# moyun/deneva

Measured on AMD Instinct MI355X. Metric: OCC-validated txns/sec, YCSB theta=0.9, higher is better.
Workload: dtype u64; 1 GPU; YCSB OCC epoch validation, 1048576 txns x 16 keys, zipf theta=0.9, 16,777,216-key table, 50% RO txns, 50% WR tuples; global_batch=1048576, keys_per_txn=16, parallelism=single GPU

## Files before the change

### deneva_amd/csrc/occ_sweep.hip

```cpp
#include <hip/hip_runtime.h>

#include <algorithm>

#include "dcc_device.h"
#include "occ_kernels.h"
#include "prep_body.h"

namespace dcc {

constexpr uint32_t LB_ACC_BITS = 34;

__device__ inline uint32_t sw_hash(uint64_t key, uint32_t log2s) {
  const uint32_t h = (uint32_t)key * 0x9E3779B1u ^ (uint32_t)(key >> 32) * 0x85EBCA77u;
  return h >> (32 - log2s);
}

__device__ inline uint32_t gtab_step(uint64_t key, uint32_t gbits, uint32_t step) {
  const uint32_t h = sw_hash(key, gbits);
  const uint32_t nbm = (1u << (gbits - 2)) - 1u;
  const uint32_t b = ((h >> 2) + (step >> 2)) & nbm;
  return 4 * b + (((h & 3u) + step) & 3u);
}
__device__ inline unsigned long long gtab_cas(uint64_t* gt, uint32_t slot, uint64_t key) {
  return atomicCAS((unsigned long long*)(gt + slot), (unsigned long long)KEY_EMPTY,
// ... 599 lines not shown
      while (true) {
        if (lds_ld(&s_stop)) {
          stopped = true;
          break;
        }
        if (lds_ld(&s_done) + SEQ_RING > k) break;
        pw++;
        __builtin_amdgcn_s_sleep(8);
      }
      if (stopped) break;
      const uint4* src = (const uint4*)(a.rec + k);
      uint4* dst = (uint4*)&ring[slot];
      uint4 v[SEQ_V4 / 64];
#pragma unroll
      for (uint32_t q = 0; q < SEQ_V4 / 64; q++) v[q] = src[q * 64 + lane];
#pragma unroll
      for (uint32_t q = 0; q < SEQ_V4 / 64; q++) dst[q * 64 + lane] = v[q];
      if (lane == 0) lds_st(&s_ready[slot], k + 1);
    }
    if (dbg && lane == 0 && pw) atomicAdd((unsigned long long*)&dbg[7], (unsigned long long)pw);
  } else if (ntiles) {
    uint32_t k = 0, cw = 0, st_it = 0;
    uint64_t st_u = 0;
    __builtin_amdgcn_s_setprio(3);
    const uint64_t cyc0 = __builtin_amdgcn_s_memtime();
    while (lds_ld(&s_ready[0]) != 1u) {
      cw++;
      __builtin_amdgcn_s_sleep(1);
    }
    uint64_t cdep, cseg[SW_RC];
    uint32_t cmeta, chdr, cpe[SW_RC], cie[SW_RC_I];
    auto read_rec = [&](const SwRec& T) {
      cdep = T.dep[lane];
      cmeta = T.meta[lane];
      chdr = T.hdr;
#pragma unroll
      for (uint32_t c = 0; c < SW_RC; c++) {
        cpe[c] = T.probe[c * 64 + lane];
        cseg[c] = T.seg[c][lane];
      }
#pragma unroll
      for (uint32_t c = 0; c < SW_RC_I; c++) cie[c] = T.ins[c * 64 + lane];
    };
    read_rec(ring[0]);
    if (ntiles > 1)
      while (lds_ld(&s_ready[1 % SEQ_RING]) != 2u) {
        cw++;
        __builtin_amdgcn_s_sleep(1);
      }
    uint32_t fl = 0, slot = 0;
    for (; k < ntiles; k++) {
      const uint32_t hdr = __builtin_amdgcn_readfirstlane(chdr);
      if (hdr & SWH_STOP) break;
      const uint64_t dep = cdep;
      const uint32_t meta = cmeta;
      uint64_t seg[SW_RC];
      uint32_t pe[SW_RC], ie[SW_RC_I];
#pragma unroll
      for (uint32_t c = 0; c < SW_RC; c++) {
        seg[c] = cseg[c];
        pe[c] = cpe[c];
      }
#pragma unroll
      for (uint32_t c = 0; c < SW_RC_I; c++) ie[c] = cie[c];
      const uint32_t kn = k + 1, sn = slot + 1 == SEQ_RING ? 0u : slot + 1;
      uint32_t h[SW_RC];
#pragma unroll
      for (uint32_t c = 0; c < SW_RC; c++) h[c] = cb_probe(cbits, pe[c]);
      read_rec(ring[sn]);
      fl = lds_ld_rlx(&s_ready[sn + 1 == SEQ_RING ? 0u : sn + 1]);
      uint64_t kv = 0;
#pragma unroll
      for (uint32_t c = 0; c < SW_RC; c++) kv |= ballot64(h[c] != 0) & seg[c];
      uint64_t K = ballot64(kv != 0);
      if (hdr & SWH_PLONG) {
        const uint32_t np = __builtin_amdgcn_readfirstlane(ring[slot].np);
        const uint32_t sp = ring[slot].pspan[lane];
        const uint32_t ps = sp & 0xFFFFu, pe2 = sp >> 16;
        const uint32_t* ovf = a.lst_ovf + (uint64_t)k * SW_OVF;
        bool kill = false;
        for (uint32_t q0 = SW_RC * 64; q0 < np; q0 += 64) {
          const uint32_t q = q0 + lane;
          uint32_t e = SW_P_NONE;
          if (q < np) e = q < SW_PL ? ring[slot].probe[q] : ld_sync(ovf + (q - SW_PL));
          kill |= seg_any(ballot64(cb_probe(cbits, e) != 0), ps, pe2, q0);
        }
        K |= ballot64(kill);
      }
      uint64_t U = ballot64((meta & (SWM_VALID | SWM_PRE)) == SWM_VALID) & ~K, M = 0;
      st_u += __builtin_popcountll(U);
      if (U) {
        const uint64_t d = ballot64((dep & U) == 0);
        M = U & d;
        U &= ~d;
        while (U) {
          const uint64_t cm = U & ballot64((dep & (M | U)) == 0);
          const uint64_t am = U & ballot64((dep & M) != 0);
          M |= cm;
          U &= ~(cm | am);
          st_it++;
        }
      }
      if (kn + 1 < ntiles)
        while (fl != kn + 2) {
          cw++;
          __builtin_amdgcn_s_sleep(1);
          fl = lds_ld_rlx(&s_ready[sn + 1 == SEQ_RING ? 0u : sn + 1]);
        }
      __atomic_signal_fence(__ATOMIC_SEQ_CST);
#pragma unroll
      for (uint32_t c = 0; c < SW_RC_I; c++) cb_insert_m(cbits, ie[c], M);
      if (hdr & SWH_ILONG) {
        const uint32_t ni = __builtin_amdgcn_readfirstlane(ring[slot].ni);
        const uint32_t* ovf = a.lst_ovf + (uint64_t)k * SW_OVF;
        for (uint32_t q0 = SW_RC_I * 64; q0 < ni; q0 += 64) {
          const uint32_t q = q0 + lane;
          uint32_t e = sw_idummy(lane);
          if (q < ni) e = q < SW_IL ? ring[slot].ins[q] : ld_sync(ovf + SW_TA + (q - SW_IL));
          cb_insert_m(cbits, e, M);
        }
      }
      s_M[k] = M;
      __hip_atomic_store(&s_done, kn, __ATOMIC_RELAXED, __HIP_MEMORY_SCOPE_WORKGROUP);
      slot = sn;
    }
    if (lane == 0) {
      s_k = k;
      lds_st(&s_stop, 1u);
      if (dbg) {
        dbg[2] = __builtin_amdgcn_s_memrealtime();
        dbg[5] = cw;
        dbg[6] = k;
        dbg[8] = __builtin_amdgcn_s_memtime() - cyc0;
        dbg[9] = st_u;
        dbg[10] = st_it;
      }
    }
  }
  __syncthreads();
  const uint32_t k = s_k;
  constexpr uint32_t WO_U = 8;
  for (uint32_t q0 = 0; q0 < k * SW_T; q0 += SEQ_B * WO_U) {
    uint32_t mt[WO_U], tid[WO_U];
#pragma unroll
    for (uint32_t u = 0; u < WO_U; u++) {
      const uint32_t q = q0 + u * SEQ_B + j;
      mt[u] = 0;
      tid[u] = 0;
      if (q < k * SW_T) {
        mt[u] = a.rec[q / SW_T].meta[q % SW_T];
        tid[u] = a.rec[q / SW_T].rtid[q % SW_T];
      }
    }
    bool cw[WO_U];
#pragma unroll
    for (uint32_t u = 0; u < WO_U; u++) {
      const uint32_t q = q0 + u * SEQ_B + j;
      cw[u] = false;
      if (mt[u] & SWM_VALID) {
        const bool com = (s_M[q / SW_T] >> (q % SW_T)) & 1ull;
        if (!(mt[u] & SWM_PRE)) a.state[tid[u]] = com ? ST_COMMIT : ST_ABORT;
        if (a.write_hasw) a.hasw[tid[u]] = (mt[u] & SWM_HASW) ? 1 : 0;
        cw[u] = com && !(mt[u] & SWM_PRE) && (mt[u] & SWM_HASW);
      }
    }
    if (a.cw_list) {
      uint64_t bm[WO_U];
      uint32_t tot = 0;
#pragma unroll
      for (uint32_t u = 0; u < WO_U; u++) {
        bm[u] = ballot64(cw[u]);
        tot += (uint32_t)__popcll(bm[u]);
      }
      uint32_t base = 0;
      if (lane == 0 && tot) base = atomicAdd(a.cw_count, tot);
      base = __shfl(base, 0);
#pragma unroll
      for (uint32_t u = 0; u < WO_U; u++) {
        if (cw[u]) a.cw_list[base + (uint32_t)__popcll(bm[u] & lanemask_lt())] = tid[u];
        base += (uint32_t)__popcll(bm[u]);
      }
    }
  }
  if (dbg) {
    __syncthreads();
    if (j == 0) dbg[3] = __builtin_amdgcn_s_memrealtime();
  }
  for (uint32_t q = j; q < k; q += SEQ_B) a.mg[q] = s_M[q];
  for (uint32_t q = j; q < nwords; q += SEQ_B) a.cbits_out[q] = 0;
  for (uint32_t q = j; q < (1u << SW_BLOOM_LOG) / 32; q += SEQ_B) a.bloom_out[q] = 0;
  if (j == 0) {
    a.lv->pos = min(k * SW_T, lim);
    a.lv->ccount = 0;
    if (dbg) dbg[4] = __builtin_amdgcn_s_memrealtime();
  }
}

__global__ __launch_bounds__(256) void k_sw_cout(SwCoutArgs a) {
  __shared__ uint32_t s_cnt[4];
  __shared__ uint32_t s_base;
  if (blockIdx.x >= a.cout_grid) {
    const uint32_t b = blockIdx.x - a.cout_grid, nb = gridDim.x - a.cout_grid;
    prep_body_hasw(a.prep_off, a.prep_n, a.prep_at, a.prep_nnz, a.hasw, a.prep_part, b, nb, a.prep_err);
    const uint4 e = make_uint4(~0u, ~0u, ~0u, ~0u);
    for (uint64_t q = (uint64_t)b * 256 + threadIdx.x; q < a.wclear_n16; q += (uint64_t)nb * 256)
      a.wclear[q] = e;
    return;
  }
  const uint32_t ab = *a.abandon;
  const uint32_t pos = a.lv->pos;
  const uint32_t m = list_len(a.m_dev, a.m_host);
  const uint32_t o0_raw = a.in.off[0];
  if (ab) return;
  if (a.skip_done && pos >= m) return;
  const uint32_t lane = lane_id(), wv = threadIdx.x >> 6;
  const uint64_t nnz = a.in.nnz;
  const uint32_t off0 = (uint32_t)min((uint64_t)o0_raw, nnz);
  const uint32_t range = (uint32_t)min((uint64_t)a.in.off[pos], nnz) - off0;
  for (uint32_t x0 = blockIdx.x * 1024; x0 < range; x0 += gridDim.x * 1024) {
    uint32_t ent[4], ap[4];
    uint64_t kx[4];
    bool c[4];
#pragma unroll
    for (uint32_t u = 0; u < 4; u++) {
      const uint32_t x = x0 + wv * 256 + u * 64 + lane;
      const bool in = x < range;
      ent[u] = in ? a.aent[x] : 0u;
      ap[u] = in ? a.apos[x] : 0u;
      kx[u] = in ? a.in.keys[off0 + x] : 0ull;
    }
    uint64_t mw[4];
#pragma unroll
    for (uint32_t u = 0; u < 4; u++) mw[u] = (ent[u] & 32u) ? a.mg[ap[u] >> 6] : 0ull;
#pragma unroll
    for (uint32_t u = 0; u < 4; u++) c[u] = (ent[u] & 32u) && ((mw[u] >> (ap[u] & 63u)) & 1ull);
    uint64_t cm[4];
    uint32_t wc = 0;
#pragma unroll
    for (uint32_t u = 0; u < 4; u++) {
      cm[u] = ballot64(c[u]);
      wc += (uint32_t)__popcll(cm[u]);
    }
    if (lane == 0) s_cnt[wv] = wc;
    __syncthreads();
    if (threadIdx.x == 0) {
      const uint32_t tot = s_cnt[0] + s_cnt[1] + s_cnt[2] + s_cnt[3];
      s_base = tot ? atomicAdd(&a.lv->ccount, tot) : 0u;
    }
    __syncthreads();
    uint32_t base = s_base;
    for (uint32_t w = 0; w < wv; w++) base += s_cnt[w];
#pragma unroll
    for (uint32_t u = 0; u < 4; u++) {
      if (c[u]) {
        const uint64_t key = kx[u];
        a.ckeys_out[base + (uint32_t)__popcll(cm[u] & lanemask_lt())] = key;
        const uint32_t id = sw_aid(ent[u]);
        if (id < SW_ID_NONE) atomicOr(&a.cbits_out[id >> 5], 1u << (id & 31u));
        uint32_t b1, b2;
        bloom_bits(key, b1, b2);
        atomicOr(&a.bloom_out[b1 >> 5], 1u << (b1 & 31));
        atomicOr(&a.bloom_out[b2 >> 5], 1u << (b2 & 31));
      }
      base += (uint32_t)__popcll(cm[u]);
    }
    __syncthreads();
  }
}


constexpr uint32_t FW = SW_CHUNK / 64;
constexpr uint32_t FK = 16;
constexpr uint32_t SW_CMP_MAXR = 4096;

__device__ inline bool c_exact(const SwFilterArgs& a, uint64_t key) {
  const uint32_t nbm = (1u << (a.gbits - 2)) - 1u;
  uint32_t b = sw_hash(key, a.gbits - 2);
  for (uint32_t q = 0; q <= nbm; q++) {
    const uint4* p = (const uint4*)(a.gtab + 4 * (uint64_t)b);
    const uint4 x = p[0], y = p[1];
    const uint32_t nib = (a.cbits[b >> 3] >> ((b & 7u) * 4u)) & 15u;
    const uint64_t v0 = ((uint64_t)x.y << 32) | x.x, v1 = ((uint64_t)x.w << 32) | x.z;
    const uint64_t v2 = ((uint64_t)y.y << 32) | y.x, v3 = ((uint64_t)y.w << 32) | y.z;
    if (v0 == key) return nib & 1u;
    if (v1 == key) return (nib >> 1) & 1u;
    if (v2 == key) return (nib >> 2) & 1u;
    if (v3 == key) return (nib >> 3) & 1u;
    if (v0 == KEY_EMPTY || v1 == KEY_EMPTY || v2 == KEY_EMPTY || v3 == KEY_EMPTY) return false;
    b = (b + 1) & nbm;
  }
  return false;
}
constexpr uint32_t F_STASH = 256;
#ifndef DCC_F_XS
#define DCC_F_XS 2048
#endif
#ifndef DCC_F_WPE
#define DCC_F_WPE 1
#endif
constexpr uint32_t F_XS = DCC_F_XS;
constexpr uint32_t F_XCAP = F_XS / 2;
constexpr uint32_t F_XBITS_LOG = 16;

__global__ __launch_bounds__(SW_CHUNK, DCC_F_WPE) void k_sw_filter(SwFilterArgs a) {
  constexpr uint32_t B = SW_CHUNK, FW = B / 64;
  constexpr uint32_t CS = F_XS;
  struct XSet {
    uint32_t bl[(1u << F_XBITS_LOG) / 32];
    uint64_t cex[F_XS];
  };
  union FSet {
    XSet x;
    uint32_t bl[(1u << SW_BLOOM_LOG) / 32];
  };
  __shared__ __attribute__((aligned(16))) FSet fs;
  uint32_t* const bl = fs.bl;
  uint64_t* const cex = fs.x.cex;
  __shared__ uint64_t s_hit[FW][SW_WA / 64];
  __shared__ uint64_t s_stash[FW][F_STASH];
  __shared__ uint32_t s_wpre[FW][SW_WA / 64];
  const uint32_t j = threadIdx.x, lane = lane_id(), wv = j >> 6;
  const uint32_t ab = *a.abandon;
  const uint32_t m = list_len(a.m_dev, a.m_host);
  const uint32_t pos = a.lv->pos;
  const uint32_t ccount = a.lv->ccount;
  if (ab) return;
  const bool X = ccount <= F_XCAP;
  uint64_t* dbg = (a.dbg && blockIdx.x < 256 && j == 0) ? a.dbg + 8 * blockIdx.x : nullptr;
  if (dbg) dbg[0] = __builtin_amdgcn_s_memrealtime();
  if (pos >= m && !a.kill_out) return;
  for (uint64_t q = (uint64_t)blockIdx.x * B + j; q < a.gclear_n;
       q += (uint64_t)gridDim.x * B) {
    a.gclear[q] = KEY_EMPTY;
    a.fw_clear[q] = ~0u;
    a.la_clear[q] = 0u;
  }
  if (pos >= m) return;
  const uint32_t n64 = (m - pos + 63) / 64;
  const uint64_t nnz = a.in.nnz;
  const uint32_t R = sw_tiles_per_wg(n64, gridDim.x);
  const uint32_t t_lo = min(blockIdx.x * R, n64), t_hi = min(t_lo + R, n64);
  if (t_lo >= t_hi) {
    if (!a.kill_out && j == 0) {
      a.bsum[blockIdx.x] = 0;
      if (a.ro_split) a.rbsum[blockIdx.x] = 0;
    }
    return;
  }
  const bool small = X;
  {
    if (!X) {
      const uint4* src = (const uint4*)a.bloom;
      uint4* dst = (uint4*)bl;
      for (uint32_t q = j; q < (1u << SW_BLOOM_LOG) / 128; q += B) dst[q] = src[q];
    } else {
      for (uint32_t q = j; q < (1u << F_XBITS_LOG) / 32; q += B) bl[q] = 0;
      for (uint32_t q = j; q < CS; q += B) cex[q] = KEY_EMPTY;
    }
  }
  __syncthreads();
  if (small) {
    for (uint32_t q = j; q < ccount; q += B) {
      const uint64_t kq = a.ckeys[q];
      lset_insert<CS>(cex, kq);
      if (X) {
        uint32_t b1, b2;
        bloom_bits(kq, b1, b2);
        b1 >>= SW_BLOOM_LOG - F_XBITS_LOG;
        atomicOr(&bl[b1 >> 5], 1u << (b1 & 31u));
      }
    }
    __syncthreads();
  }
  if (dbg) dbg[1] = __builtin_amdgcn_s_memrealtime();
  uint64_t* hit = s_hit[wv];
  uint64_t* stash = s_stash[wv];
  uint64_t wsum = 0, rsum = 0;
  uint32_t ns = 0, ne = 0, ntid = 0, nst = 0, nhw = 1;
  auto prefetch = [&](uint32_t wt) {
    const uint32_t pc = min(pos + wt * 64 + lane, m - 1);
    ns = a.in.off[pc];
    ne = a.in.off[pc + 1];
    ntid = a.in.tid ? a.in.tid[pc] : pc;
    nst = a.cand_state ? a.state[pc] : 0u;
    if (a.ro_split) nhw = a.hasw[pc];
  };
  if (t_lo + wv < t_hi) prefetch(t_lo + wv);
  for (uint32_t wt = t_lo + wv; wt < t_hi; wt += FW) {
    const uint32_t p = pos + wt * 64 + lane;
    const bool valid = p < m;
    uint32_t s = 0, e = 0, tid = 0;
    bool cand = false, ro = false;
    if (valid) {
      s = (uint32_t)min((uint64_t)ns, nnz);
      e = (uint32_t)min((uint64_t)ne, nnz);
      if (e < s) e = s;
      tid = ntid;
      cand = nst == ST_UNDECIDED;
      ro = nhw == 0;
    }
    bool pref = false;
    const uint64_t vm = ballot64(valid);
    const uint32_t A0 = vm ? __shfl(s, 0) : 0u;
    const uint32_t A1 = wave_reduce<MaxOp<uint32_t>>(valid ? e : 0u);
    uint32_t span = A1 > A0 ? A1 - A0 : 0u;
    if (span > SW_WA) {
      if (lane == 0) atomicOr(a.err, ERR_TILE);
      span = 0;
    }
    const uint32_t nw = (span + 63) / 64;
    uint32_t npos = 0;
    bool bad_key = false;
    for (uint32_t b0 = 0; b0 < span; b0 += 64 * FK) {
      uint64_t key[FK];
#pragma unroll
      for (uint32_t u = 0; u < FK; u++) {
        const uint32_t xr = b0 + 64 * u + lane;
        const uint32_t x = A0 + (xr < span ? xr : 0u);
        key[u] = a.in.keys[x];
      }
      if (!pref) {
        pref = true;
        if (wt + FW < t_hi) prefetch(wt + FW);
      }
#pragma unroll
      for (uint32_t u = 0; u < FK; u++) {
        const uint32_t xr = b0 + 64 * u + lane;
        if (b0 + 64 * u >= span) continue;
        const bool in = xr < span;
        bad_key |= in && key[u] == KEY_EMPTY;
        bool h;
        uint32_t b1, b2;
        bloom_bits(key[u], b1, b2);
        if (X) {
          b1 >>= SW_BLOOM_LOG - F_XBITS_LOG;
          h = in && ((bl[b1 >> 5] >> (b1 & 31u)) & 1u) != 0;
        } else {
          const uint32_t wa = bl[b1 >> 5], wb = bl[b2 >> 5];
          h = in && (((wa >> (b1 & 31u)) & (wb >> (b2 & 31u)) & 1u) != 0);
        }
        const uint64_t hb = ballot64(h);
        if (h) {
          const uint32_t ci = npos + (uint32_t)__popcll(hb & lanemask_lt());
          if (ci < F_STASH) stash[ci] = key[u];
        }
        npos += (uint32_t)__popcll(hb);
        if (lane == 0) hit[(b0 >> 6) + u] = hb;
      }
    }
    if (!pref && wt + FW < t_hi) prefetch(wt + FW);
    if (ballot64(bad_key) && lane == 0) atomicOr(a.err, ERR_KEY);
    if (dbg && wt == t_lo) dbg[2] = __builtin_amdgcn_s_memrealtime();
    const uint32_t rlo = s - A0, rlen = e - s;
    const bool ok = valid && (rlen == 0 || (uint64_t)rlo + rlen <= span);
    bool killed = false;
    {
      {
        const uint32_t pw = lane < nw ? (uint32_t)__popcll(hit[lane]) : 0u;
        uint32_t ptot;
        const uint32_t pre = wave_excl<AddOp<uint32_t>>(pw, ptot);
        if (lane < nw) s_wpre[wv][lane] = pre;
      }
      if (cand && ok && rlen) {
        for (uint32_t x = rlo; x < rlo + rlen; x++) {
          const uint32_t nx = range_next(hit, x, rlo + rlen);
          if (nx >= rlo + rlen) break;
          const uint32_t ci = s_wpre[wv][nx >> 6] +
                              (uint32_t)__popcll(hit[nx >> 6] & ((1ull << (nx & 63)) - 1ull));
          const uint64_t kx = ci < F_STASH ? stash[ci] : a.in.keys[A0 + nx];
          if (small ? lset_find<CS>(cex, kx) : c_exact(a, kx)) {
            killed = true;
            break;
          }
          x = nx;
        }
      }
    }
    if (dbg && wt == t_lo) dbg[3] = __builtin_amdgcn_s_memrealtime();
    if (dbg) dbg[6]++;
    if (a.kill_out) {
      const uint64_t km = ballot64(valid && killed);
      if (lane == 0) a.kill_out[wt] = km;
      continue;
    }
    if (killed) a.state[tid] = ST_ABORT;
    if (cand && ok && rlen == 0) a.state[tid] = ST_COMMIT;
    const bool surv = cand && ok && rlen && !killed;
    const uint64_t sm = ballot64(surv);
    const uint64_t acc = wave_reduce<AddOp<uint64_t>>(surv ? rlen : 0u);
    const uint64_t cnt = ((uint64_t)__popcll(sm) << LB_ACC_BITS) | acc;
    wsum += cnt;
    if (lane == 0) {
      a.sflag[wt] = sm;
      a.tcount[wt] = cnt;
    }
    if (a.ro_split) {
      const uint64_t rm = ballot64(surv && ro);
      const uint64_t racc = wave_reduce<AddOp<uint64_t>>(surv && ro ? rlen : 0u);
      const uint64_t rc = ((uint64_t)__popcll(rm) << LB_ACC_BITS) | racc;
      rsum += rc;
      if (lane == 0) {
        a.rflag[wt] = rm;
        a.rtcount[wt] = rc;
      }
    }
    if (dbg && wt == t_lo) {
      __builtin_amdgcn_s_waitcnt(0);
      dbg[4] = __builtin_amdgcn_s_memrealtime();
    }
  }
  if (a.kill_out) return;
  __shared__ unsigned long long s_bs[FW][2];
  if (lane == 0) {
    s_bs[wv][0] = wsum;
    s_bs[wv][1] = rsum;
  }
  __syncthreads();
  if (j == 0) {
    uint64_t t = 0, r = 0;
    for (uint32_t w = 0; w < FW; w++) {
      t += s_bs[w][0];
      r += s_bs[w][1];
    }
    a.bsum[blockIdx.x] = t;
    if (a.ro_split) a.rbsum[blockIdx.x] = r;
  }
  if (dbg) {
    __builtin_amdgcn_s_waitcnt(0);
    dbg[5] = __builtin_amdgcn_s_memrealtime();
  }
}

__global__ __launch_bounds__(SW_CHUNK) void k_sw_apply(SwFilterArgs a) {
  const uint32_t lane = lane_id(), wv = threadIdx.x >> 6;
  if (*a.abandon) return;
  const uint32_t m = list_len(a.m_dev, a.m_host);
  const uint32_t pos = a.lv->pos;
  if (pos >= m) return;
  const uint32_t n64 = (m - pos + 63) / 64;
  const uint64_t nnz = a.in.nnz;
  const uint32_t R = sw_tiles_per_wg(n64, gridDim.x);
  const uint32_t t_lo = min(blockIdx.x * R, n64), t_hi = min(t_lo + R, n64);
  uint64_t wsum = 0, rsum = 0;
  for (uint32_t wt = t_lo + wv; wt < t_hi; wt += SW_CHUNK / 64) {
    const uint32_t p = pos + wt * 64 + lane;
    uint64_t kw = 0;
    for (uint32_t r = 0; r < a.kill_ranks; r++) kw |= a.kill_in[r * a.kill_stride + wt];
    const bool kill = (kw >> lane) & 1ull;
    bool surv = false, ro = false;
    uint32_t len = 0;
    if (p < m) {
      const uint32_t tid = a.in.tid ? a.in.tid[p] : p;
      const bool cand = a.cand_state ? a.state[p] == ST_UNDECIDED : true;
      const uint32_t s = (uint32_t)min((uint64_t)a.in.off[p], nnz);
      const uint32_t e = (uint32_t)min((uint64_t)a.in.off[p + 1], nnz);
      len = e > s ? e - s : 0u;
      if (cand && kill) a.state[tid] = ST_ABORT;
      surv = cand && !kill;
      ro = a.ro_split && a.hasw[tid] == 0;
    }
    const uint64_t sm = ballot64(surv);
    const uint64_t acc = wave_reduce<AddOp<uint64_t>>(surv ? len : 0u);
    const uint64_t cnt = ((uint64_t)__popcll(sm) << LB_ACC_BITS) | acc;
    wsum += cnt;
    if (lane == 0) {
      a.sflag[wt] = sm;
      a.tcount[wt] = cnt;
    }
    if (a.ro_split) {
      const uint64_t rm = ballot64(surv && ro);
      const uint64_t racc = wave_reduce<AddOp<uint64_t>>(surv && ro ? len : 0u);
      const uint64_t rc = ((uint64_t)__popcll(rm) << LB_ACC_BITS) | racc;
      rsum += rc;
      if (lane == 0) {
        a.rflag[wt] = rm;
        a.rtcount[wt] = rc;
      }
    }
  }
  __shared__ unsigned long long s_bs[SW_CHUNK / 64][2];
  if (lane == 0) {
    s_bs[wv][0] = wsum;
    s_bs[wv][1] = rsum;
  }
  __syncthreads();
  if (threadIdx.x == 0) {
    uint64_t t = 0, r = 0;
    for (uint32_t w = 0; w < SW_CHUNK / 64; w++) {
      t += s_bs[w][0];
      r += s_bs[w][1];
    }
    a.bsum[blockIdx.x] = t;
    if (a.ro_split) a.rbsum[blockIdx.x] = r;
  }
}

constexpr uint32_t SG_T = 1024;
__global__ __launch_bounds__(SG_T) void k_sw_sg_scan(const uint32_t* tid, const uint32_t* m_dev, uint32_t p_max,
                                                     const uint32_t* full_off, uint64_t full_nnz, uint32_t* soff,
                                                     uint32_t* err) {
  __shared__ uint32_t s_w[SG_T / 64];
  __shared__ uint32_t s_carry;
  const uint32_t P = min(p_max, *m_dev);
  if (threadIdx.x == 0) s_carry = 0;
  __syncthreads();
  for (uint32_t q0 = 0; q0 < P; q0 += SG_T) {
    const uint32_t q = q0 + threadIdx.x;
    uint32_t len = 0;
    if (q < P) {
      const uint32_t t = tid[q];
      const uint64_t s = min((uint64_t)full_off[t], full_nnz), e = min((uint64_t)full_off[t + 1], full_nnz);
      len = e > s ? (uint32_t)(e - s) : 0u;
      if (len > MAX_TXN_LEN) {
        atomicOr(err, ERR_OFFSETS);
        len = 0;
      }
    }
    uint32_t tot;
    const uint32_t ex = s_carry + block_excl<SG_T / 64, AddOp<uint32_t>>(len, s_w, tot);
    if (q < P) soff[q] = ex;
    __syncthreads();
    if (threadIdx.x == SG_T - 1) s_carry = ex + len;
    __syncthreads();
  }
  if (threadIdx.x == 0) soff[P] = s_carry;
}
__global__ __launch_bounds__(256) void k_sw_sg_copy(const uint32_t* tid, const uint32_t* m_dev, uint32_t p_max,
                                                    const uint32_t* full_off, const uint64_t* full_keys,
                                                    const uint8_t* full_at, uint64_t full_nnz, const uint32_t* soff,
                                                    uint64_t* skeys, uint8_t* sat) {
  const uint32_t P = min(p_max, *m_dev), sl = threadIdx.x & 15u;
  for (uint32_t q = (blockIdx.x * 256 + threadIdx.x) >> 4; q < P; q += gridDim.x * 16) {
    const uint32_t t = tid[q], o = soff[q], len = soff[q + 1] - o;
    const uint64_t s = min((uint64_t)full_off[t], full_nnz);
    for (uint32_t x = sl; x < len; x += 16) {
      skeys[o + x] = full_keys[s + x];
      sat[o + x] = full_at[s + x];
    }
  }
}

__global__ void k_sw_share(const uint32_t* m_dev, uint32_t m_host, const uint32_t* abandon,
                           const uint32_t* off, uint32_t p_max, uint32_t rank, uint32_t* cnt) {
  const uint32_t m = m_dev ? *m_dev : m_host;
  const uint32_t P = min(p_max, m);
  cnt[0] = m;
  cnt[1] = *abandon;
  cnt[2 + rank] = m ? off[P] - off[0] : 0u;
}

__global__ __launch_bounds__(256) void k_sw_export(SwList in, uint32_t P, uint32_t* rec) {
  const uint64_t nnz = in.nnz;
  const uint32_t off0 = (uint32_t)min((uint64_t)in.off[0], nnz);
  for (uint32_t t = blockIdx.x * 4 + (threadIdx.x >> 6); t < P; t += gridDim.x * 4) {
    const uint32_t s = (uint32_t)min((uint64_t)in.off[t], nnz);
    const uint32_t e = (uint32_t)min((uint64_t)in.off[t + 1], nnz);
    for (uint32_t x = s + lane_id(); x < e; x += 64) {
      const uint64_t k = in.keys[x];
      uint32_t* r = rec + 3ull * (x - off0);
      r[0] = (uint32_t)k;
      r[1] = (uint32_t)(k >> 32);
      r[2] = t | ((uint32_t)(in.acctype[x] & 3u) << 30);
    }
  }
}

__global__ __launch_bounds__(256) void k_sw_mcount(const uint32_t* rec, uint32_t n, uint32_t P,
                                                   uint32_t* cnt) {
  for (uint32_t i = blockIdx.x * 256 + threadIdx.x; i < n; i += gridDim.x * 256) {
    const uint32_t t = rec[3ull * i + 2] & 0x3FFFFFFFu;
    if (t < P) atomicAdd(&cnt[t], 1u);
  }
}
__global__ __launch_bounds__(1024) void k_sw_mscan(uint32_t* cnt, uint32_t P, uint32_t* off,
                                                   uint32_t* cur) {
  __shared__ uint32_t s_w[16];
  __shared__ uint32_t s_carry;
  const uint32_t j = threadIdx.x, lane = lane_id(), wv = j >> 6;
  if (j == 0) s_carry = 0;
  __syncthreads();
  for (uint32_t c0 = 0; c0 < P; c0 += 1024) {
    const uint32_t t = c0 + j;
    const uint32_t v = t < P ? cnt[t] : 0u;
    uint32_t tot;
    const uint32_t ex = wave_excl<AddOp<uint32_t>>(v, tot);
    if (lane == 0) s_w[wv] = tot;
    __syncthreads();
    uint32_t base = s_carry;
    for (uint32_t w = 0; w < wv; w++) base += s_w[w];
    if (t < P) {
      off[t] = base + ex;
      cur[t] = base + ex;
    }
    __syncthreads();
    if (j == 0) {
      uint32_t all = 0;
      for (uint32_t w = 0; w < 16; w++) all += s_w[w];
      s_carry += all;
    }
    __syncthreads();
  }
  if (j == 0) off[P] = s_carry;
}
__global__ __launch_bounds__(256) void k_sw_mscatter(const uint32_t* rec, uint32_t n, uint32_t P,
                                                     uint32_t* cur, uint64_t* keys,
                                                     uint8_t* at) {
  for (uint32_t i = blockIdx.x * 256 + threadIdx.x; i < n; i += gridDim.x * 256) {
    const uint32_t w2 = rec[3ull * i + 2];
    if ((w2 & 0x3FFFFFFFu) >= P) continue;
    const uint32_t q = atomicAdd(&cur[w2 & 0x3FFFFFFFu], 1u);
    keys[q] = ((uint64_t)rec[3ull * i + 1] << 32) | rec[3ull * i];
    at[q] = (uint8_t)(w2 >> 30);
  }
}

__global__ __launch_bounds__(SW_CHUNK) void k_sw_compact(SwFilterArgs a) {
  const uint32_t lane = lane_id(), wv = threadIdx.x >> 6;
  const uint32_t ab = *a.abandon;
  const uint32_t m = list_len(a.m_dev, a.m_host);
  const uint32_t pos = a.lv->pos;
  if (ab && ab != a.level + 1) return;
  if (pos >= m) return;
  const uint32_t n64 = (m - pos + 63) / 64;
  const uint64_t nnz = a.in.nnz;
  const uint32_t R = sw_tiles_per_wg(n64, a.nblocks);
  const uint32_t t_lo = min(blockIdx.x * R, n64), t_hi = min(t_lo + R, n64);
  if (t_lo >= t_hi && blockIdx.x) return;
  uint64_t* dbg = (a.cdbg && blockIdx.x == 0 && threadIdx.x == 0) ? a.cdbg : nullptr;
  if (dbg) dbg[0] = __builtin_amdgcn_s_memrealtime();
  __shared__ unsigned long long s_tb[SW_CMP_MAXR];
  __shared__ unsigned long long s_part[SW_CHUNK / 64][4];
  __shared__ uint32_t s_split, s_rnext;
  if (R > SW_CMP_MAXR) {
    if (threadIdx.x == 0) atomicOr(a.err, ERR_TILE);
    return;
  }
  {
    uint64_t pre = 0, all = 0, rpre = 0, rall = 0;
    constexpr uint32_t TU = 4;
    for (uint32_t q0 = threadIdx.x; q0 < a.nblocks; q0 += SW_CHUNK * TU) {
      uint64_t v[TU], r[TU];
#pragma unroll
      for (uint32_t u = 0; u < TU; u++) {
        const uint32_t q = q0 + u * SW_CHUNK;
        v[u] = q < a.nblocks ? a.bsum[q] : 0ull;
        r[u] = (a.ro_split && q < a.nblocks) ? a.rbsum[q] : 0ull;
      }
#pragma unroll
      for (uint32_t u = 0; u < TU; u++) {
        const uint32_t q = q0 + u * SW_CHUNK;
        all += v[u];
        rall += r[u];
        if (q < blockIdx.x) {
          pre += v[u];
          rpre += r[u];
        }
      }
    }
    pre = wave_reduce<AddOp<uint64_t>>(pre);
    all = wave_reduce<AddOp<uint64_t>>(all);
    rpre = wave_reduce<AddOp<uint64_t>>(rpre);
    rall = wave_reduce<AddOp<uint64_t>>(rall);
    if (lane == 0) {
      s_part[wv][0] = pre;
      s_part[wv][1] = all;
      s_part[wv][2] = rpre;
      s_part[wv][3] = rall;
    }
    __syncthreads();
    if (threadIdx.x == 0) {
      uint64_t p0 = 0, a0 = 0, rp = 0, ra = 0;
      for (uint32_t w = 0; w < SW_CHUNK / 64; w++) {
        p0 += s_part[w][0];
        a0 += s_part[w][1];
        rp += s_part[w][2];
        ra += s_part[w][3];
      }
      const uint32_t tot = (uint32_t)(a0 >> LB_ACC_BITS);
      const uint32_t in_n = m - pos;
      const bool handoff =
          tot > a.abandon_min && (uint64_t)tot * a.abandon_den > (uint64_t)in_n * a.abandon_num;
      const bool split = a.ro_split && !handoff;
      s_split = split ? 1u : 0u;
      s_part[0][0] = split ? p0 - rp : p0;
      s_rnext = (uint32_t)(rp >> LB_ACC_BITS);
      if (blockIdx.x == 0) {
        const uint64_t keep = split ? a0 - ra : a0;
        const uint32_t kt = (uint32_t)(keep >> LB_ACC_BITS);
        const uint64_t acc = keep & ((1ull << LB_ACC_BITS) - 1);
        a.lv_next->m = kt;
        a.lv_next->acc = (uint32_t)acc;
        a.off_out[kt] = (uint32_t)acc;
        if (a.ro_split) *a.ro_count = split ? (uint32_t)(ra >> LB_ACC_BITS) : 0u;
        if (handoff) atomicMax(a.abandon_out, a.level + 1);
      }
    }
    __syncthreads();
  }
  const bool split = s_split != 0;
  if (dbg) dbg[1] = __builtin_amdgcn_s_memrealtime();
  if (wv == 0) {
    uint64_t run = s_part[0][0];
    for (uint32_t c0 = t_lo; c0 < t_hi; c0 += 64) {
      const uint32_t q = c0 + lane;
      const uint64_t v = (q < t_hi ? a.tcount[q] : 0ull) - ((split && q < t_hi) ? a.rtcount[q] : 0ull);
      uint64_t tot;
      const uint64_t ex = wave_excl<AddOp<uint64_t>>(v, tot);
      if (q < t_hi) s_tb[q - t_lo] = run + ex;
      run += tot;
    }
  }
  __syncthreads();
  if (dbg) dbg[2] = __builtin_amdgcn_s_memrealtime();
  constexpr uint32_t CB = 4;
  for (uint32_t w0 = t_lo + wv; w0 < t_hi; w0 += FW * CB) {
    uint64_t wordv[CB], rwordv[CB];
    uint32_t sv[CB], ev[CB], tv[CB];
#pragma unroll
    for (uint32_t i = 0; i < CB; i++) {
      const uint32_t wt = w0 + FW * i;
      const uint32_t pc = min(pos + min(wt, n64 - 1) * 64 + lane, m - 1);
      wordv[i] = wt < t_hi ? a.sflag[wt] : 0ull;
      rwordv[i] = (split && wt < t_hi) ? a.rflag[wt] : 0ull;
      sv[i] = a.in.off[pc];
      ev[i] = a.in.off[pc + 1];
      tv[i] = a.in.tid ? a.in.tid[pc] : pc;
    }
#pragma unroll
    for (uint32_t i = 0; i < CB; i++) {
      const uint32_t wt = w0 + FW * i;
// ... 203 lines not shown
```

Before: 5.879 billion txns/s.

## Template filter loop on X mode with DPP reductions and batched hit recording

Moves the per-tile filter loop into a function templated on the small-set versus bloom mode. Each round now loads keys with clamped addresses and records per-round hit masks and stash prefixes through writelane, so lane 0 no longer writes per round and the separate prefix scan is dropped. Wave reductions now use DPP plus readlane, and the small-set path uses a cheaper single-hash bit index. The restructuring adds code size and register pressure, and the new hash may change the false-positive rate; a numpy script is added to measure that rate.

Result: faster. 6.366 billion txns/s (median of 5 runs) (+8.3%).

```diff
diff --git a/deneva_amd/csrc/occ_sweep.hip b/deneva_amd/csrc/occ_sweep.hip
--- a/deneva_amd/csrc/occ_sweep.hip
+++ b/deneva_amd/csrc/occ_sweep.hip
@@ -925,6 +925,195 @@
 constexpr uint32_t F_XCAP = F_XS / 2;
 constexpr uint32_t F_XBITS_LOG = 16;
 
+
+__device__ inline uint32_t xset_bit(uint64_t key) {
+  return (((uint32_t)key ^ (uint32_t)(key >> 32)) * 0x9E3779B1u) >> (32 - F_XBITS_LOG);
+}
+
+extern "C" __device__ int dcc_writelane(int v, int lane, int old) __asm("llvm.amdgcn.writelane.i32");
+
+template <typename Op>
+__device__ inline uint32_t wave_all_dpp(uint32_t v) {
+  v = Op::f(v, (uint32_t)__builtin_amdgcn_update_dpp(0, (int)v, 0xB1, 0xF, 0xF, false));
+  v = Op::f(v, (uint32_t)__builtin_amdgcn_update_dpp(0, (int)v, 0x4E, 0xF, 0xF, false));
+  v = Op::f(v, (uint32_t)__builtin_amdgcn_update_dpp(0, (int)v, 0x141, 0xF, 0xF, false));
+  v = Op::f(v, (uint32_t)__builtin_amdgcn_update_dpp(0, (int)v, 0x140, 0xF, 0xF, false));
+  const uint32_t r0 = __builtin_amdgcn_readlane((int)v, 0), r1 = __builtin_amdgcn_readlane((int)v, 16);
+  const uint32_t r2 = __builtin_amdgcn_readlane((int)v, 32), r3 = __builtin_amdgcn_readlane((int)v, 48);
+  return Op::f(Op::f(r0, r1), Op::f(r2, r3));
+}
+struct DppAdd {
+  static __device__ uint32_t f(uint32_t a, uint32_t b) { return a + b; }
+};
+struct DppMax {
+  static __device__ uint32_t f(uint32_t a, uint32_t b) { return a > b ? a : b; }
+};
+
+struct FWave {
+  uint64_t* hit;
+  uint32_t* wpre;
+  uint64_t* stash;
+};
+
+template <bool X, uint32_t NR>
+__device__ inline bool filter_rounds(const uint64_t* kp, uint32_t rem, const uint32_t* bl,
+                                     const FWave& L, uint32_t w0, uint32_t lane, uint32_t& npos) {
+  constexpr uint32_t G = X ? NR : (NR < 8 ? NR : 8);
+  uint32_t lane8 = 8 * lane;
+  asm volatile("" : "+v"(lane8));
+  const uint32_t last8 = 8 * (rem - 1);
+  uint64_t key[NR];
+#pragma unroll
+  for (uint32_t u = 0; u < NR; u++)
+    key[u] = *(const uint64_t*)((const char*)kp + min(512 * u + lane8, last8));
+  bool bad = false;
+  uint32_t wl = 0, wh = 0, pre = 0;
+#pragma unroll
+  for (uint32_t g = 0; g < NR; g += G) {
+    uint32_t i1[G], i2[X ? 1 : G], w1[G], w2[X ? 1 : G];
+#pragma unroll
+    for (uint32_t v = 0; v < G; v++) {
+      const uint64_t k = key[g + v];
+      bad |= k == KEY_EMPTY;
+      if (X) {
+        i1[v] = xset_bit(k);
+        w1[v] = bl[i1[v] >> 5];
+      } else {
+        bloom_bits(k, i1[v], i2[v]);
+        w1[v] = bl[i1[v] >> 5];
+        w2[v] = bl[i2[v] >> 5];
+      }
+    }
+#pragma unroll
+    for (uint32_t v = 0; v < G; v++) {
+      const uint32_t u = g + v;
+      uint32_t in = lane < (rem > 64 * u ? rem - 64 * u : 0u) ? 1u : 0u;
+      asm volatile("" : "+v"(in));
+      uint32_t bit = w1[v] >> (i1[v] & 31u);
+      if (!X) bit &= w2[v] >> (i2[v] & 31u);
+      const bool h = (bit & in) != 0;
+      const uint64_t hb = __builtin_amdgcn_ballot_w64(h);
+      const uint32_t hlo = (uint32_t)hb, hhi = (uint32_t)(hb >> 32);
+      const int ci = (int)__builtin_amdgcn_mbcnt_hi(hhi, __builtin_amdgcn_mbcnt_lo(hlo, 0u));
+      if (h && ci < (int)F_STASH - (int)npos) (L.stash + npos)[ci] = key[u];
+      wl = dcc_writelane(hlo, u, wl);
+      wh = dcc_writelane(hhi, u, wh);
+      pre = dcc_writelane(npos, u, pre);
+      npos += (uint32_t)__popcll(hb);
+    }
+  }
+  if (lane < NR) {
+    L.hit[w0 + lane] = ((uint64_t)wh << 32) | wl;
+    L.wpre[w0 + lane] = pre;
+  }
+  return bad;
+}
+
+template <bool X>
+__device__ inline void filter_tiles(const SwFilterArgs& a, const uint32_t* bl, const uint64_t* cex,
+                                    const FWave& L, uint32_t wv, uint32_t pos, uint32_t m,
+                                    uint32_t t_lo, uint32_t t_hi, uint64_t* dbg, uint64_t& wsum,
+                                    uint64_t& rsum) {
+  constexpr uint32_t CS = F_XS;
+  const uint32_t lane = lane_id();
+  const uint64_t nnz = a.in.nnz;
+  uint32_t ns = 0, ne = 0, ntid = 0, nst = 0, nhw = 1;
+  auto prefetch = [&](uint32_t wt) {
+    const uint32_t pc = min(pos + wt * 64 + lane, m - 1);
+    ns = a.in.off[pc];
+    ne = a.in.off[pc + 1];
+    ntid = a.in.tid ? a.in.tid[pc] : pc;
+    nst = a.cand_state ? a.state[pc] : 0u;
+    if (a.ro_split) nhw = a.hasw[pc];
+  };
+  prefetch(t_lo + wv);
+  for (uint32_t wt = t_lo + wv; wt < t_hi; wt += FW) {
+    const uint32_t p = pos + wt * 64 + lane;
+    const bool valid = p < m;
+    uint32_t s = 0, e = 0, tid = 0;
+    bool cand = false, ro = false;
+    if (valid) {
+      s = (uint32_t)min((uint64_t)ns, nnz);
+      e = (uint32_t)min((uint64_t)ne, nnz);
+      if (e < s) e = s;
+      tid = ntid;
+      cand = nst == ST_UNDECIDED;
+      ro = nhw == 0;
+    }
+    prefetch(wt + FW);
+    const uint64_t vm = ballot64(valid);
+    const uint32_t A0 = vm ? __builtin_amdgcn_readfirstlane(s) : 0u;
+    const uint32_t A1 = wave_all_dpp<DppMax>(valid ? e : 0u);
+    const uint32_t sp = A1 > A0 ? A1 - A0 : 0u;
+    const uint32_t span = sp > SW_WA ? 0u : sp;
+    if (sp > SW_WA && lane == 0) atomicOr(a.err, ERR_TILE);
+    uint32_t npos = 0;
+    bool bad_key = false;
+    for (uint32_t b0 = 0; b0 < span;) {
+      const uint64_t* kp = a.in.keys + A0 + b0;
+      const uint32_t rem = span - b0;
+      if (rem > 64 * (FK / 2)) {
+        bad_key |= filter_rounds<X, FK>(kp, rem, bl, L, b0 >> 6, lane, npos);
+        b0 += 64 * FK;
+      } else {
+        bad_key |= filter_rounds<X, FK / 2>(kp, rem, bl, L, b0 >> 6, lane, npos);
+        b0 += 64 * (FK / 2);
+      }
+    }
+    if (ballot64(bad_key) && lane == 0) atomicOr(a.err, ERR_KEY);
+    if (dbg && wt == t_lo && lane == 0) dbg[2] = __builtin_amdgcn_s_memrealtime();
+    const uint32_t rlo = s - A0, rlen = e - s;
+    const bool ok = valid && (rlen == 0 || (uint64_t)rlo + rlen <= span);
+    bool killed = false;
+    if (cand && ok && rlen) {
+      for (uint32_t x = rlo; x < rlo + rlen; x++) {
+        const uint32_t nx = range_next(L.hit, x, rlo + rlen);
+        if (nx >= rlo + rlen) break;
+        const uint32_t ci = L.wpre[nx >> 6] +
+                            (uint32_t)__popcll(L.hit[nx >> 6] & ((1ull << (nx & 63)) - 1ull));
+        const uint64_t kx = ci < F_STASH ? L.stash[ci] : a.in.keys[A0 + nx];
+        if (X ? lset_find<CS>(cex, kx) : c_exact(a, kx)) {
+          killed = true;
+          break;
+        }
+        x = nx;
+      }
+    }
+    if (dbg && wt == t_lo && lane == 0) dbg[3] = __builtin_amdgcn_s_memrealtime();
+    if (dbg && lane == 0) dbg[6]++;
+    if (a.kill_out) {
+      const uint64_t km = ballot64(valid && killed);
+      if (lane == 0) a.kill_out[wt] = km;
+      continue;
+    }
+    if (killed) a.state[tid] = ST_ABORT;
+    if (cand && ok && rlen == 0) a.state[tid] = ST_COMMIT;
+    const bool surv = cand && ok && rlen && !killed;
+    const uint64_t sm = ballot64(surv);
+    const uint64_t acc = wave_all_dpp<DppAdd>(surv ? rlen : 0u);
+    const uint64_t cnt = ((uint64_t)__popcll(sm) << LB_ACC_BITS) | acc;
+    wsum += cnt;
+    if (lane == 0) {
+      a.sflag[wt] = sm;
+      a.tcount[wt] = cnt;
+    }
+    if (a.ro_split) {
+      const uint64_t rm = ballot64(surv && ro);
+      const uint64_t racc = wave_all_dpp<DppAdd>(surv && ro ? rlen : 0u);
+      const uint64_t rc = ((uint64_t)__popcll(rm) << LB_ACC_BITS) | racc;
+      rsum += rc;
+      if (lane == 0) {
+        a.rflag[wt] = rm;
+        a.rtcount[wt] = rc;
+      }
+    }
+    if (dbg && wt == t_lo) {
+      __builtin_amdgcn_s_waitcnt(0);
+      if (lane == 0) dbg[4] = __builtin_amdgcn_s_memrealtime();
+    }
+  }
+}
+
 __global__ __launch_bounds__(SW_CHUNK, DCC_F_WPE) void k_sw_filter(SwFilterArgs a) {
   constexpr uint32_t B = SW_CHUNK, FW = B / 64;
   constexpr uint32_t CS = F_XS;
@@ -942,15 +1131,16 @@
   __shared__ uint64_t s_hit[FW][SW_WA / 64];
   __shared__ uint64_t s_stash[FW][F_STASH];
   __shared__ uint32_t s_wpre[FW][SW_WA / 64];
-  const uint32_t j = threadIdx.x, lane = lane_id(), wv = j >> 6;
+  const uint32_t j = threadIdx.x, lane = lane_id();
+  const uint32_t wv = __builtin_amdgcn_readfirstlane(j >> 6);
   const uint32_t ab = *a.abandon;
   const uint32_t m = list_len(a.m_dev, a.m_host);
   const uint32_t pos = a.lv->pos;
   const uint32_t ccount = a.lv->ccount;
   if (ab) return;
   const bool X = ccount <= F_XCAP;
-  uint64_t* dbg = (a.dbg && blockIdx.x < 256 && j == 0) ? a.dbg + 8 * blockIdx.x : nullptr;
-  if (dbg) dbg[0] = __builtin_amdgcn_s_memrealtime();
+  uint64_t* dbg = (a.dbg && blockIdx.x < 256 && wv == 0) ? a.dbg + 8 * blockIdx.x : nullptr;
+  if (dbg && lane == 0) dbg[0] = __builtin_amdgcn_s_memrealtime();
   if (pos >= m && !a.kill_out) return;
   for (uint64_t q = (uint64_t)blockIdx.x * B + j; q < a.gclear_n;
        q += (uint64_t)gridDim.x * B) {
@@ -960,7 +1150,6 @@
   }
   if (pos >= m) return;
   const uint32_t n64 = (m - pos + 63) / 64;
-  const uint64_t nnz = a.in.nnz;
   const uint32_t R = sw_tiles_per_wg(n64, gridDim.x);
   const uint32_t t_lo = min(blockIdx.x * R, n64), t_hi = min(t_lo + R, n64);
   if (t_lo >= t_hi) {
@@ -970,168 +1159,30 @@
     }
     return;
   }
-  const bool small = X;
-  {
-    if (!X) {
-      const uint4* src = (const uint4*)a.bloom;
-      uint4* dst = (uint4*)bl;
-      for (uint32_t q = j; q < (1u << SW_BLOOM_LOG) / 128; q += B) dst[q] = src[q];
-    } else {
-      for (uint32_t q = j; q < (1u << F_XBITS_LOG) / 32; q += B) bl[q] = 0;
-      for (uint32_t q = j; q < CS; q += B) cex[q] = KEY_EMPTY;
-    }
-  }
-  __syncthreads();
-  if (small) {
+  if (!X) {
+    const uint4* src = (const uint4*)a.bloom;
+    uint4* dst = (uint4*)bl;
+    for (uint32_t q = j; q < (1u << SW_BLOOM_LOG) / 128; q += B) dst[q] = src[q];
+    __syncthreads();
+  } else {
+    for (uint32_t q = j; q < (1u << F_XBITS_LOG) / 32; q += B) bl[q] = 0;
+    for (uint32_t q = j; q < CS; q += B) cex[q] = KEY_EMPTY;
+    __syncthreads();
     for (uint32_t q = j; q < ccount; q += B) {
       const uint64_t kq = a.ckeys[q];
       lset_insert<CS>(cex, kq);
-      if (X) {
-        uint32_t b1, b2;
-        bloom_bits(kq, b1, b2);
-        b1 >>= SW_BLOOM_LOG - F_XBITS_LOG;
-        atomicOr(&bl[b1 >> 5], 1u << (b1 & 31u));
-      }
-    }
-    __syncthreads();
-  }
-  if (dbg) dbg[1] = __builtin_amdgcn_s_memrealtime();
-  uint64_t* hit = s_hit[wv];
-  uint64_t* stash = s_stash[wv];
+      const uint32_t b1 = xset_bit(kq);
+      atomicOr(&bl[b1 >> 5], 1u << (b1 & 31u));
+    }
+    __syncthreads();
+  }
+  if (dbg && lane == 0) dbg[1] = __builtin_amdgcn_s_memrealtime();
+  const FWave L{s_hit[wv], s_wpre[wv], s_stash[wv]};
   uint64_t wsum = 0, rsum = 0;
-  uint32_t ns = 0, ne = 0, ntid = 0, nst = 0, nhw = 1;
-  auto prefetch = [&](uint32_t wt) {
-    const uint32_t pc = min(pos + wt * 64 + lane, m - 1);
-    ns = a.in.off[pc];
-    ne = a.in.off[pc + 1];
-    ntid = a.in.tid ? a.in.tid[pc] : pc;
-    nst = a.cand_state ? a.state[pc] : 0u;
-    if (a.ro_split) nhw = a.hasw[pc];
-  };
-  if (t_lo + wv < t_hi) prefetch(t_lo + wv);
-  for (uint32_t wt = t_lo + wv; wt < t_hi; wt += FW) {
-    const uint32_t p = pos + wt * 64 + lane;
-    const bool valid = p < m;
-    uint32_t s = 0, e = 0, tid = 0;
-    bool cand = false, ro = false;
-    if (valid) {
-      s = (uint32_t)min((uint64_t)ns, nnz);
-      e = (uint32_t)min((uint64_t)ne, nnz);
-      if (e < s) e = s;
-      tid = ntid;
-      cand = nst == ST_UNDECIDED;
-      ro = nhw == 0;
-    }
-    bool pref = false;
-    const uint64_t vm = ballot64(valid);
-    const uint32_t A0 = vm ? __shfl(s, 0) : 0u;
-    const uint32_t A1 = wave_reduce<MaxOp<uint32_t>>(valid ? e : 0u);
-    uint32_t span = A1 > A0 ? A1 - A0 : 0u;
-    if (span > SW_WA) {
-      if (lane == 0) atomicOr(a.err, ERR_TILE);
-      span = 0;
-    }
-    const uint32_t nw = (span + 63) / 64;
-    uint32_t npos = 0;
-    bool bad_key = false;
-    for (uint32_t b0 = 0; b0 < span; b0 += 64 * FK) {
-      uint64_t key[FK];
-#pragma unroll
-      for (uint32_t u = 0; u < FK; u++) {
-        const uint32_t xr = b0 + 64 * u + lane;
-        const uint32_t x = A0 + (xr < span ? xr : 0u);
-        key[u] = a.in.keys[x];
-      }
-      if (!pref) {
-        pref = true;
-        if (wt + FW < t_hi) prefetch(wt + FW);
-      }
-#pragma unroll
-      for (uint32_t u = 0; u < FK; u++) {
-        const uint32_t xr = b0 + 64 * u + lane;
-        if (b0 + 64 * u >= span) continue;
-        const bool in = xr < span;
-        bad_key |= in && key[u] == KEY_EMPTY;
-        bool h;
-        uint32_t b1, b2;
-        bloom_bits(key[u], b1, b2);
-        if (X) {
-          b1 >>= SW_BLOOM_LOG - F_XBITS_LOG;
-          h = in && ((bl[b1 >> 5] >> (b1 & 31u)) & 1u) != 0;
-        } else {
-          const uint32_t wa = bl[b1 >> 5], wb = bl[b2 >> 5];
-          h = in && (((wa >> (b1 & 31u)) & (wb >> (b2 & 31u)) & 1u) != 0);
-        }
-        const uint64_t hb = ballot64(h);
-        if (h) {
-          const uint32_t ci = npos + (uint32_t)__popcll(hb & lanemask_lt());
-          if (ci < F_STASH) stash[ci] = key[u];
-        }
-        npos += (uint32_t)__popcll(hb);
-        if (lane == 0) hit[(b0 >> 6) + u] = hb;
-      }
-    }
-    if (!pref && wt + FW < t_hi) prefetch(wt + FW);
-    if (ballot64(bad_key) && lane == 0) atomicOr(a.err, ERR_KEY);
-    if (dbg && wt == t_lo) dbg[2] = __builtin_amdgcn_s_memrealtime();
-    const uint32_t rlo = s - A0, rlen = e - s;
-    const bool ok = valid && (rlen == 0 || (uint64_t)rlo + rlen <= span);
-    bool killed = false;
-    {
-      {
-        const uint32_t pw = lane < nw ? (uint32_t)__popcll(hit[lane]) : 0u;
-        uint32_t ptot;
-        const uint32_t pre = wave_excl<AddOp<uint32_t>>(pw, ptot);
-        if (lane < nw) s_wpre[wv][lane] = pre;
-      }
-      if (cand && ok && rlen) {
-        for (uint32_t x = rlo; x < rlo + rlen; x++) {
-          const uint32_t nx = range_next(hit, x, rlo + rlen);
-          if (nx >= rlo + rlen) break;
-          const uint32_t ci = s_wpre[wv][nx >> 6] +
-                              (uint32_t)__popcll(hit[nx >> 6] & ((1ull << (nx & 63)) - 1ull));
-          const uint64_t kx = ci < F_STASH ? stash[ci] : a.in.keys[A0 + nx];
-          if (small ? lset_find<CS>(cex, kx) : c_exact(a, kx)) {
-            killed = true;
-            break;
-          }
-          x = nx;
-        }
-      }
-    }
-    if (dbg && wt == t_lo) dbg[3] = __builtin_amdgcn_s_memrealtime();
-    if (dbg) dbg[6]++;
-    if (a.kill_out) {
-      const uint64_t km = ballot64(valid && killed);
-      if (lane == 0) a.kill_out[wt] = km;
-      continue;
-    }
-    if (killed) a.state[tid] = ST_ABORT;
-    if (cand && ok && rlen == 0) a.state[tid] = ST_COMMIT;
-    const bool surv = cand && ok && rlen && !killed;
-    const uint64_t sm = ballot64(surv);
-    const uint64_t acc = wave_reduce<AddOp<uint64_t>>(surv ? rlen : 0u);
-    const uint64_t cnt = ((uint64_t)__popcll(sm) << LB_ACC_BITS) | acc;
-    wsum += cnt;
-    if (lane == 0) {
-      a.sflag[wt] = sm;
-      a.tcount[wt] = cnt;
-    }
-    if (a.ro_split) {
-      const uint64_t rm = ballot64(surv && ro);
-      const uint64_t racc = wave_reduce<AddOp<uint64_t>>(surv && ro ? rlen : 0u);
-      const uint64_t rc = ((uint64_t)__popcll(rm) << LB_ACC_BITS) | racc;
-      rsum += rc;
-      if (lane == 0) {
-        a.rflag[wt] = rm;
-        a.rtcount[wt] = rc;
-      }
-    }
-    if (dbg && wt == t_lo) {
-      __builtin_amdgcn_s_waitcnt(0);
-      dbg[4] = __builtin_amdgcn_s_memrealtime();
-    }
-  }
+  if (X)
+    filter_tiles<true>(a, bl, cex, L, wv, pos, m, t_lo, t_hi, dbg, wsum, rsum);
+  else
+    filter_tiles<false>(a, bl, cex, L, wv, pos, m, t_lo, t_hi, dbg, wsum, rsum);
   if (a.kill_out) return;
   __shared__ unsigned long long s_bs[FW][2];
   if (lane == 0) {
@@ -1148,7 +1199,7 @@
     a.bsum[blockIdx.x] = t;
     if (a.ro_split) a.rbsum[blockIdx.x] = r;
   }
-  if (dbg) {
+  if (dbg && lane == 0) {
     __builtin_amdgcn_s_waitcnt(0);
     dbg[5] = __builtin_amdgcn_s_memrealtime();
   }
diff --git a/profiles/r07/filter_rounds/fp_rate.py b/profiles/r07/filter_rounds/fp_rate.py
--- /dev/null
+++ b/profiles/r07/filter_rounds/fp_rate.py
@@ -0,0 +1,40 @@
+import sys
+import numpy as np
+import os
+ROOT = os.path.join(os.path.dirname(os.path.abspath(__file__)), "..", "..", "..")
+sys.path.insert(0, ROOT); sys.path.insert(0, os.path.join(ROOT, "tests"))
+import deneva_amd as d
+import _oracle as orc
+
+def old_idx(k):
+    lo = (k & 0xFFFFFFFF).astype(np.uint64); hi = (k >> np.uint64(32)).astype(np.uint64)
+    h = ((lo * 0x9E3779B1) ^ (hi * 0x85EBCA77)) & 0xFFFFFFFF
+    return (h >> np.uint64(16)).astype(np.int64)
+
+def new_idx(k):
+    lo = (k & 0xFFFFFFFF).astype(np.uint64); hi = (k >> np.uint64(32)).astype(np.uint64)
+    h = ((lo ^ hi) * 0x9E3779B1) & 0xFFFFFFFF
+    return (h >> np.uint64(16)).astype(np.int64)
+
+def rate(b, name, P=1024):
+    rc = orc.occ(b)[0]
+    off = np.asarray(b.offsets, np.int64); keys = np.asarray(b.keys, np.uint64); at = np.asarray(b.acctype)
+    owner = np.repeat(np.arange(b.n_txn), np.diff(off))
+    commit = rc == rc[0]
+    WR = at.max() if len(np.unique(at)) == 2 else None
+    wmask = (owner < P) & commit[owner] & (at == WR)
+    C = np.unique(keys[wmask])
+    rest = keys[off[P]:]
+    inC = np.isin(rest, C)
+    for nm, f in (("old", old_idx), ("new", new_idx)):
+        bm = np.zeros(1 << 16, bool); bm[f(C)] = True
+        pos = bm[f(rest)]
+        fp = (pos & ~inC).sum()
+        print(f"{name} {nm}: |C| {len(C)}, bits set {bm.sum()}, accesses {len(rest)}, positives {pos.sum()}, "
+              f"false positives {fp} = {100.0 * fp / len(rest):.3f} % of accesses "
+              f"({100.0 * fp / max(1, (~inC).sum()):.3f} % of non-members)")
+
+print("acctype values", np.unique(np.asarray(d.gen_ycsb(n_txn=1024, zipf_theta=0.9).acctype)))
+rate(d.gen_ycsb(n_txn=1 << 20, zipf_theta=0.9), "headline")
+rate(d.gen_ycsb(n_txn=1 << 20, zipf_theta=0.99, seed=0xD3E7A002), "C5")
+rate(d.gen_tpcc(n_txn=262144, num_wh=128), "C3 tpcc")
```
